# yuanqing-wang/stag

Hardware: NVIDIA B200
Metric: GEdge-samples/s fused stochastic SpMM fwd+bwd (higher is better)
Workload: dtype f32

## Files before the change

stag_b200/csrc/gemm_tcgen05.cu:

```cuda
#include <cuda.h>
#include <stdlib.h>

#include "common.cuh"

namespace stag {

constexpr int GM = 128;
constexpr int GK = 32;
constexpr int GTHREADS = 128;

__device__ __forceinline__ uint32_t smem_u32(const void* p) { return (uint32_t)__cvta_generic_to_shared(p); }

__device__ __forceinline__ float to_tf32(float x) {
  uint32_t y;
  asm("cvt.rna.tf32.f32 %0, %1;" : "=r"(y) : "f"(x));
  return __uint_as_float(y);
}

__device__ __forceinline__ uint64_t make_desc(uint32_t saddr) {
  return (uint64_t)((saddr & 0x3FFFFu) >> 4) | (1ull << 16) | (64ull << 32) | (1ull << 46) | (2ull << 61);
}

__device__ __forceinline__ uint32_t make_idesc(int n) {
  return (1u << 4) | (2u << 7) | (2u << 10) | ((uint32_t)(n >> 3) << 17) | ((uint32_t)(GM >> 4) << 24);
}

__device__ __forceinline__ void mma_tf32(uint32_t tmem_d, uint64_t da, uint64_t db, uint32_t idesc, uint32_t accumulate) {
  asm volatile(
      "{\n\t.reg .pred p;\n\tsetp.ne.b32 p, %4, 0;\n\t"
      "tcgen05.mma.cta_group::1.kind::tf32 [%0], %1, %2, %3, p;\n\t}"
      ::"r"(tmem_d), "l"(da), "l"(db), "r"(idesc), "r"(accumulate)
      : "memory");
}
// ... 490 lines not shown
          const uint32_t s = st.i, l = lo.i;
          mbar_wait_s(FULL(s), st.par);
          if (!lo_first) mbar_wait_s(LO_FREE(l), lo.par ^ 1u);
          st.next();
          lo.next();
          if (lo.i == 0) lo_first = false;
          const uint32_t hi_s = st0 + s * G2_TILE, lo_s = lo0 + l * G2_TILE;
          uint32_t x[8][4];
#pragma unroll
          for (int j = 0; j < 8; ++j) {
            const int idx = lane + 32 * j, r = 32 * w + (idx >> 3), ch = idx & 7;
            const uint32_t o = (uint32_t)r * 128u + (uint32_t)((ch ^ (r & 7)) << 4);
            asm volatile("ld.shared.v4.b32 {%0,%1,%2,%3}, [%4];" : "=r"(x[j][0]), "=r"(x[j][1]), "=r"(x[j][2]), "=r"(x[j][3]) : "r"(hi_s + o));
          }
#pragma unroll
          for (int j = 0; j < 8; ++j) {
            const int idx = lane + 32 * j, r = 32 * w + (idx >> 3), ch = idx & 7;
            const uint32_t o = (uint32_t)r * 128u + (uint32_t)((ch ^ (r & 7)) << 4);
            float l4[4];
#pragma unroll
            for (int t = 0; t < 4; ++t) l4[t] = to_tf32(__uint_as_float(x[j][t]) - __uint_as_float(x[j][t] & 0xFFFFE000u));
            asm volatile("st.shared.v4.f32 [%0], {%1,%2,%3,%4};" ::"r"(lo_s + o), "f"(l4[0]), "f"(l4[1]), "f"(l4[2]), "f"(l4[3]) : "memory");
          }
          asm volatile("fence.proxy.async.shared::cta;" ::: "memory");
          __syncwarp();
          if (lane == 0) mbar_arrive_s(READY(s));
        }
      }
    }
  }
  asm volatile("tcgen05.fence::before_thread_sync;" ::: "memory");
  __syncthreads();
  if (warp == 0) asm volatile("tcgen05.dealloc.cta_group::1.sync.aligned.b32 %0, %1;" ::"r"(tmem_d), "r"(2u * p.ncol) : "memory");
}

typedef CUresult (*EncodeTiledFn)(CUtensorMap*, CUtensorMapDataType, cuuint32_t, void*, const cuuint64_t*, const cuuint64_t*,
                                  const cuuint32_t*, const cuuint32_t*, CUtensorMapInterleave, CUtensorMapSwizzle,
                                  CUtensorMapL2promotion, CUtensorMapFloatOOBfill);
static EncodeTiledFn encode_tiled() {
  static EncodeTiledFn fn = []() -> EncodeTiledFn {
    void* f = nullptr;
    cudaDriverEntryPointQueryResult q;
    if (cudaGetDriverEntryPoint("cuTensorMapEncodeTiled", &f, cudaEnableDefault, &q) != cudaSuccess || q != cudaDriverEntryPointSuccess)
      return nullptr;
    return (EncodeTiledFn)f;
  }();
  return fn;
}

}

using namespace stag;

extern "C" size_t stag_gemm_workspace_bytes(int64_t M, int32_t Nout, int32_t K) {
  (void)M; (void)Nout; (void)K;
  return 0;
}

extern "C" int stag_gemm_tcgen05(const float* a, int64_t lda, const float* wt, int64_t ldw, int64_t M, int32_t Nout,
                                 int32_t K, const float* row_scale, const float* bias, int act, float* out,
                                 int64_t ldo, void* ws, size_t ws_bytes, void* stream_) {
  (void)ws; (void)ws_bytes;
  cudaStream_t stream = (cudaStream_t)stream_;
  STAG_CHECK_ARG(M >= 0 && Nout > 0 && K > 0, "stag_gemm_tcgen05: bad sizes M=%lld N=%d K=%d", (long long)M, Nout, K);
  if (M == 0) return STAG_OK;
  STAG_CHECK_ARG(a && wt && out, "stag_gemm_tcgen05: null argument");
  STAG_CHECK_ARG(lda >= K && ldw >= K && ldo >= Nout, "stag_gemm_tcgen05: leading dimensions too small");
  STAG_CHECK_ARG(act == 0 || act == 1, "stag_gemm_tcgen05: act must be 0 (none) or 1 (relu)");
  if (Nout > 256) {
    set_error("stag_gemm_tcgen05: Nout=%d > 256 output columns per tile are not supported", Nout);
    return STAG_EUNSUPPORTED;
  }
  {
    const int npad2 = (Nout + 15) / 16 * 16, nkb2 = (K + GK - 1) / GK;
    static const char* force1 = getenv("STAG_GEMM_FORM");
    const bool ok = lda % 4 == 0 && (((uintptr_t)a) & 15) == 0 && (size_t)npad2 * nkb2 * 128 * 2 <= 128 * 1024 &&
                    M * lda < (1ll << 40) && !(force1 && atoi(force1) == 1) && encode_tiled() != nullptr;
    if (ok) {
      alignas(64) CUtensorMap tmap;
      const cuuint64_t gdim[2] = {(cuuint64_t)K, (cuuint64_t)M};
// ... 71 lines not shown
```

stag_b200/csrc/spmm.cu:

```cuda
#include <stdlib.h>
#include "common.cuh"
#include "noise.cuh"
#include "param_finalize.cuh"

#ifndef STAG_PACK2
#define STAG_PACK2 1
#endif

namespace stag {

constexpr int AGG_THREADS = 256;
constexpr int AGG_WARPS = AGG_THREADS / 32;

struct AggParams {
  const int32_t* indptr;
  const int32_t* indices;
  const int32_t* eid;
  const int32_t* hub_rows;
  const int32_t* hub_seg_ptr;
  const int32_t* row_order;
  const int32_t* items;
  const int32_t* erow;
  const int32_t* eidf;
  const int4* rec;
  int num_items;
  uint32_t rk[2 * kPhiloxRounds];
  uint32_t kf;
  int num_hubs, num_hub_segs;
  int N;
  int64_t ncols;
  int64_t E;
  const float* x;
  int64_t ldx, x_ss;
  const float* gscale;
  const float* rscale;
// ... 2139 lines not shown
```

stag_b200/csrc/spmm_wq.cuh:

```cuda
#pragma once

namespace stag {

constexpr int WQ_GROUPS = 32, WQ_EPR = 4;
constexpr int WQ_NBUF = 4;
constexpr uint32_t WQ_REC_STRIDE = WQ_NBUF * WQ_EPR * 16 + 16;
constexpr uint32_t WQ_ROW_STRIDE = WQ_NBUF * WQ_EPR * 4 + 4;
__host__ __device__ constexpr uint32_t wq_rec_bytes(int nw) { return (uint32_t)(8 * nw) * WQ_REC_STRIDE; }
__host__ __device__ constexpr uint32_t wq_row_bytes(int nw) { return ((uint32_t)(8 * nw) * WQ_ROW_STRIDE + 15u) & ~15u; }
__host__ __device__ constexpr uint32_t wq_smem(int nw) { return 2 * 128 * 128 + wq_rec_bytes(nw) + wq_row_bytes(nw) + 1024; }

__device__ __forceinline__ void tc_ldtm_16x256b_x8(uint32_t taddr, uint32_t (&v)[32]) {
  asm volatile(
      "tcgen05.ld.sync.aligned.16x256b.x8.b32 "
      "{%0, %1, %2, %3, %4, %5, %6, %7, %8, %9, %10, %11, %12, %13, %14, %15, "
      "%16, %17, %18, %19, %20, %21, %22, %23, %24, %25, %26, %27, %28, %29, %30, %31}, [%32];"
      : "=r"(v[0]), "=r"(v[1]), "=r"(v[2]), "=r"(v[3]), "=r"(v[4]), "=r"(v[5]), "=r"(v[6]), "=r"(v[7]),
        "=r"(v[8]), "=r"(v[9]), "=r"(v[10]), "=r"(v[11]), "=r"(v[12]), "=r"(v[13]), "=r"(v[14]), "=r"(v[15]),
        "=r"(v[16]), "=r"(v[17]), "=r"(v[18]), "=r"(v[19]), "=r"(v[20]), "=r"(v[21]), "=r"(v[22]), "=r"(v[23]),
        "=r"(v[24]), "=r"(v[25]), "=r"(v[26]), "=r"(v[27]), "=r"(v[28]), "=r"(v[29]), "=r"(v[30]), "=r"(v[31])
      : "r"(taddr)
      : "memory");
}
__device__ __forceinline__ void tc_ldtm_wait32(uint32_t (&v)[32]) {
  asm volatile("tcgen05.wait::ld.sync.aligned;"
               : "+r"(v[0]), "+r"(v[1]), "+r"(v[2]), "+r"(v[3]), "+r"(v[4]), "+r"(v[5]), "+r"(v[6]), "+r"(v[7]),
                 "+r"(v[8]), "+r"(v[9]), "+r"(v[10]), "+r"(v[11]), "+r"(v[12]), "+r"(v[13]), "+r"(v[14]), "+r"(v[15]),
                 "+r"(v[16]), "+r"(v[17]), "+r"(v[18]), "+r"(v[19]), "+r"(v[20]), "+r"(v[21]), "+r"(v[22]), "+r"(v[23]),
                 "+r"(v[24]), "+r"(v[25]), "+r"(v[26]), "+r"(v[27]), "+r"(v[28]), "+r"(v[29]), "+r"(v[30]), "+r"(v[31])
               :
               : "memory");
}
__device__ __forceinline__ void tc_ldtm_16x256b_x4(uint32_t taddr, uint32_t (&v)[16]) {
  asm volatile(
      "tcgen05.ld.sync.aligned.16x256b.x4.b32 "
      "{%0, %1, %2, %3, %4, %5, %6, %7, %8, %9, %10, %11, %12, %13, %14, %15}, [%16];"
      : "=r"(v[0]), "=r"(v[1]), "=r"(v[2]), "=r"(v[3]), "=r"(v[4]), "=r"(v[5]), "=r"(v[6]), "=r"(v[7]),
        "=r"(v[8]), "=r"(v[9]), "=r"(v[10]), "=r"(v[11]), "=r"(v[12]), "=r"(v[13]), "=r"(v[14]), "=r"(v[15])
      : "r"(taddr)
      : "memory");
}
__device__ __forceinline__ void tc_ldtm_wait16(uint32_t (&v)[16]) {
  asm volatile("tcgen05.wait::ld.sync.aligned;"
               : "+r"(v[0]), "+r"(v[1]), "+r"(v[2]), "+r"(v[3]), "+r"(v[4]), "+r"(v[5]), "+r"(v[6]), "+r"(v[7]),
                 "+r"(v[8]), "+r"(v[9]), "+r"(v[10]), "+r"(v[11]), "+r"(v[12]), "+r"(v[13]), "+r"(v[14]), "+r"(v[15])
               :
               : "memory");
}
__device__ __forceinline__ void ldg256(const char* src, float4& a, float4& b) {
  asm volatile("ld.global.nc.v8.f32 {%0, %1, %2, %3, %4, %5, %6, %7}, [%8];"
               : "=f"(a.x), "=f"(a.y), "=f"(a.z), "=f"(a.w), "=f"(b.x), "=f"(b.y), "=f"(b.z), "=f"(b.w)
               : "l"(src));
}
__device__ __forceinline__ void stg256cs(char* dst, const float2* v) {
  asm volatile("st.global.cs.v8.f32 [%0], {%1, %2, %3, %4, %5, %6, %7, %8};" ::"l"(dst), "f"(v[0].x), "f"(v[0].y), "f"(v[1].x),
               "f"(v[1].y), "f"(v[2].x), "f"(v[2].y), "f"(v[3].x), "f"(v[3].y)
               : "memory");
}

template <int NW, int XB, bool DB, int MINB, int GMODE = 0, bool LATE_REC = false>
__global__ void __launch_bounds__(32 * NW, MINB) agg_wh_quad_kernel(const AggParams p) {
  constexpr int NCH = 8 / NW;
  constexpr int NU = 2 * NCH;
  constexpr int NBLK = 32 / NW;
  static_assert(NW == 4 || NW == 8, "4 or 8 warps");
  static_assert(NU % XB == 0, "ring slots must be round-invariant");
  extern __shared__ __align__(1024) unsigned char tc_raw[];
  __shared__ uint64_t mma_bar[2];
  __shared__ uint32_t tmem_base_s;
  __shared__ int maxn_s[NW];
  __shared__ int arrive_cnt[2];
  constexpr uint32_t TM_COLS = DB ? 256u : 128u;
  const uint32_t sm0 = ((uint32_t)__cvta_generic_to_shared(tc_raw) + 1023u) & ~1023u;
  const uint32_t h_s = sm0, at_s = sm0 + 128 * 128;
  const int tid = threadIdx.x, warp = tid >> 5, lane = tid & 31;
  const int wq = warp & 3;
  const int ch0 = NW == 8 ? warp >> 2 : 0;
  const int jq = lane >> 2, q = lane & 3;
  const uint32_t rec_base = at_s + 128 * 128, row_base = rec_base + wq_rec_bytes(NW);
  const uint32_t rec_g = rec_base + (uint32_t)(8 * warp + jq) * WQ_REC_STRIDE;
  const uint32_t row_g = row_base + (uint32_t)(8 * warp + jq) * WQ_ROW_STRIDE;
  const uint32_t bar_s = (uint32_t)__cvta_generic_to_shared(mma_bar);
  constexpr uint32_t rmask = WQ_NBUF * WQ_EPR - 1;

  if (warp == 0) {
    asm volatile("tcgen05.alloc.cta_group::1.sync.aligned.shared::cta.b32 [%0], %1;" ::"r"(
                     (uint32_t)__cvta_generic_to_shared(&tmem_base_s)),
                 "r"(TM_COLS)
                 : "memory");
    asm volatile("tcgen05.relinquish_alloc_permit.cta_group::1.sync.aligned;" ::: "memory");
  }
  if (tid == 0) {
    arrive_cnt[0] = arrive_cnt[1] = 0;
    tc_mbar_init(bar_s, 1);
    tc_mbar_init(bar_s + 8, 1);
    asm volatile("fence.mbarrier_init.release.cluster;" ::: "memory");
  }
  for (int n = tid; n < 128; n += 32 * NW) {
    const int kk = n >> 3, qq = (n >> 1) & 3, bb = n & 1;
    const int c = 32 * (kk >> 2) + 8 * qq + 2 * (kk & 3) + bb;
    for (int ch = 0; ch < 8; ++ch) {
      uint32_t wv[4];
#pragma unroll
      for (int w4 = 0; w4 < 4; ++w4) {
        uint32_t word = 0;
#pragma unroll
        for (int b = 0; b < 4; ++b) {
          const int k = ch * 16 + w4 * 4 + b;
          word |= ((__popc(c & k) & 1) ? 0xB8u : 0x38u) << (8 * b);
        }
        wv[w4] = word;
      }
      sts128(h_s + (uint32_t)n * 128u + (uint32_t)((ch ^ (n & 7)) << 4), make_uint4(wv[0], wv[1], wv[2], wv[3]));
    }
  }
  for (uint32_t o = (uint32_t)tid * 16u; o < 128u * 128u; o += 32u * NW * 16u) sts128(at_s + o, make_uint4(0u, 0u, 0u, 0u));
  asm volatile("fence.proxy.async.shared::cta;" ::: "memory");
  asm volatile("tcgen05.fence::before_thread_sync;" ::: "memory");
  __syncthreads();
  asm volatile("tcgen05.fence::after_thread_sync;" ::: "memory");
  const uint32_t tmem0 = tmem_base_s;
  const uint32_t idesc = (1u << 4) | ((uint32_t)(128 >> 3) << 17) | ((uint32_t)(128 >> 4) << 24);
  const uint64_t h_desc = tc_desc(h_s), a_desc = tc_desc(at_s);
  const PhiloxKey key = live_key(p);
  uint32_t mma_count = 0;

  const int G = p.D >> 7;
  const int n_items = p.num_hub_segs + p.num_items;
  const int IG = (n_items + WQ_GROUPS - 1) / WQ_GROUPS;
  const int64_t total = (int64_t)IG * p.S * G;
  const uint32_t ldxb = (uint32_t)p.ldx * 4u, ldo4 = (uint32_t)p.ldo * 4u;
  const int rb = NW == 8 ? 16 * (warp >> 2) : 0;
  const uint32_t mk_rec = rec_base + (uint32_t)(8 * warp + (lane >> 3)) * WQ_REC_STRIDE + 4u;
  const uint32_t mk_row = at_s + (uint32_t)(32 * wq + rb + (lane >> 3)) * 128u;

  __shared__ int item_s;
  int* const queue = reinterpret_cast<int*>(const_cast<int4*>(p.rec) + p.E);
  if (tid == 0) item_s = atomicAdd(queue, 1);
  __syncthreads();
  for (;;) {
    const int64_t item = item_s;
    if (item >= total) break;
    const int64_t outer = item / IG;
    const int gi = (int)(item - outer * IG) * WQ_GROUPS + 8 * wq + jq;
    const int cg = (int)(outer % G), s = (int)(outer / G);
    int e0 = 0, e1 = 0, part_slot = -1;
    if (gi < p.num_hub_segs) {
      int lo = 0, hi = p.num_hubs;
      while (hi - lo > 1) {
        const int mid = (lo + hi) >> 1;
        if (__ldg(p.hub_seg_ptr + mid) <= gi) lo = mid; else hi = mid;
      }
      const int row = __ldg(p.hub_rows + lo);
      const int k = gi - __ldg(p.hub_seg_ptr + lo);
      e0 = __ldg(p.indptr + row) + k * kHubSegment;
      e1 = min(e0 + kHubSegment, __ldg(p.indptr + row + 1));
      part_slot = gi;
    } else if (gi < n_items) {
      const int4 it = __ldg(reinterpret_cast<const int4*>(p.items) + (gi - p.num_hub_segs));
      e0 = it.z;
      e1 = it.w >= 0 ? it.w : it.z;
    }
    const int nedges = e1 - e0;
    const int rowlim = part_slot < 0 ? nedges : 0;
    int maxn = nedges;
#pragma unroll
    for (int o = 16; o > 0; o >>= 1) maxn = max(maxn, __shfl_xor_sync(0xffffffffu, maxn, o));
    __syncthreads();
    if (lane == 0) maxn_s[warp] = maxn;
    if (tid == 0) item_s = atomicAdd(queue, 1);
    __syncthreads();
    maxn = max(max(maxn_s[0], maxn_s[1]), max(maxn_s[2], maxn_s[3]));
    const int rounds = (maxn + WQ_EPR - 1) / WQ_EPR;
    if (rounds == 0) continue;

    const char* xcb = reinterpret_cast<const char*>(p.x + (int64_t)s * p.x_ss + cg * 128 + 64 * ch0 + 8 * q);
    char* outs = reinterpret_cast<char*>(p.out + (int64_t)s * p.out_ss + cg * 128 + 64 * ch0 + 8 * q);
    const uint32_t smp = (uint32_t)(p.sample_base + s);
    const uint32_t blk = (uint32_t)(8 * cg + (lane & 7));
    const int4* recp = p.rec + e0;
    const int32_t* rowp = p.erow + e0;
    float2 acc[8 * NCH];
#pragma unroll
    for (int i = 0; i < 8 * NCH; ++i) acc[i] = make_float2(0.f, 0.f);
    float4 xb[XB][8];

    auto fetch_chunk = [&](int r) {
      const int e = WQ_EPR * r + q;
      const uint32_t pos = (uint32_t)e & rmask;
      const bool off = e >= nedges;
      cp_async16(rec_g + pos * 16u, recp + (off ? 0 : e), off);
      cp_async4(row_g + pos * 4u, rowp + (off ? 0 : e), off);
    };
    auto make_bytes = [&](int r) {
      uint32_t eid[NBLK];
#pragma unroll
      for (int i = 0; i < NBLK; ++i) {
        const int k = (rb + 4 * i) >> 3;
        const uint32_t pos = (uint32_t)(WQ_EPR * r + k) & rmask;
        eid[i] = (uint32_t)lds32(mk_rec + (uint32_t)(4 * (i & 1)) * WQ_REC_STRIDE + (pos << 4));
      }
      uint4 v[NBLK];
#pragma unroll
      for (int i = 0; i < NBLK; ++i) {
        v[i] = philox_rk(blk, eid[i] & 0x7fffffffu, smp, key.c3, p);
        v[i].x = (v[i].x & kWhAnd) | kWhOr; v[i].y = (v[i].y & kWhAnd) | kWhOr;
        v[i].z = (v[i].z & kWhAnd) | kWhOr; v[i].w = (v[i].w & kWhAnd) | kWhOr;
      }
#pragma unroll
      for (int i = 0; i < NBLK; ++i) {
        const int sw = ((lane >> 3) + 4 * (i & 1)) & 7;
        sts128(mk_row + (uint32_t)(4 * i) * 128u + (uint32_t)(((lane & 7) ^ sw) << 4), v[i]);
      }
    };
    auto issue_mma = [&]() {
      const uint32_t buf = DB ? (mma_count & 1u) : 0u;
#pragma unroll
      for (int ks = 0; ks < 4; ++ks)
        tc_mma_f8(tmem0 + buf * 128u, a_desc + (uint64_t)(2 * ks), h_desc + (uint64_t)(2 * ks), idesc, ks != 0);
      asm volatile("tcgen05.commit.cta_group::1.mbarrier::arrive::one.shared::cluster.b64 [%0];" ::"r"(bar_s + 8u * (mma_count & 1u))
                   : "memory");
    };
    auto bytes_and_mma = [&](int r) {
      make_bytes(r);
      asm volatile("fence.proxy.async.shared::cta;" ::: "memory");
      asm volatile("tcgen05.fence::before_thread_sync;" ::: "memory");
      __syncwarp();
      if (lane == 0) {
        uint32_t old;
        const uint32_t cnt_s = (uint32_t)__cvta_generic_to_shared(&arrive_cnt[mma_count & 1u]);
        asm volatile("atom.acq_rel.cta.shared::cta.add.u32 %0, [%1], 1;" : "=r"(old) : "r"(cnt_s) : "memory");
        if (old == NW - 1) {
          asm volatile("st.relaxed.cta.shared::cta.u32 [%0], %1;" ::"r"(cnt_s), "r"(0u) : "memory");
          asm volatile("tcgen05.fence::after_thread_sync;" ::: "memory");
          issue_mma();
        }
      }
      ++mma_count;
    };
    auto load_half = [&](uint32_t un, int chl, float4* dst) {
      const char* src = xcb + (uint64_t)un * ldxb + 256 * chl;
      ldg256(src, dst[0], dst[1]);
      ldg256(src + 128, dst[2], dst[3]);
    };
    auto neighbours = [&](int r, uint32_t (&un)[4]) {
#pragma unroll
      for (int k4 = 0; k4 < 4; ++k4) un[k4] = (uint32_t)lds32(rec_g + (((uint32_t)(WQ_EPR * r + k4) & rmask) << 4));
    };

    fetch_chunk(0);
    fetch_chunk(1);
    cp_async_commit();
    cp_async_wait<0>();
    __syncwarp();
    bytes_and_mma(0);
    uint32_t un1[4];
    {
      uint32_t un0[4];
      neighbours(0, un0);
#pragma unroll
      for (int u = 0; u < XB; ++u) {
        load_half(un0[2 * (u / NCH)], u % NCH, xb[u]);
        load_half(un0[2 * (u / NCH) + 1], u % NCH, xb[u] + 4);
      }
    }

    for (int r = 0; r < rounds; ++r) {
      cp_async_wait<0>();
      __syncwarp();
      fetch_chunk(r + 2);
      cp_async_commit();
      int4 rc4[4];
      uint32_t ro4[4];
      auto read_records = [&]() {
#pragma unroll
        for (int k4 = 0; k4 < 4; ++k4) rc4[k4] = lds128(rec_g + (((uint32_t)(WQ_EPR * r + k4) & rmask) << 4));
#pragma unroll
        for (int k4 = 0; k4 < 4; ++k4) ro4[k4] = (uint32_t)lds32(row_g + (((uint32_t)(WQ_EPR * r + k4) & rmask) << 2));
        neighbours(r + 1, un1);
      };
      if (!LATE_REC) read_records();
      const uint32_t done = mma_count - 1u;
      tc_mbar_wait(bar_s + 8u * (done & 1u), (done >> 1) & 1u);
      asm volatile("tcgen05.fence::after_thread_sync;" ::: "memory");
      const uint32_t taddr = tmem0 + ((uint32_t)(32 * wq) << 16) + (DB ? (done & 1u) * 128u : 0u) + (uint32_t)(64 * ch0);
      if (DB && r + 1 < rounds) bytes_and_mma(r + 1);
      if (LATE_REC) read_records();
#pragma unroll
      for (int u = 0; u < NU; ++u) {
        const int hf = u / NCH, chl = u % NCH;
        uint32_t z[32];
        tc_ldtm_16x256b_x8(taddr + ((uint32_t)(16 * hf) << 16) + (uint32_t)(64 * chl), z);
        float4* xu = xb[u % XB];
        tc_ldtm_wait32(z);
#pragma unroll
        for (int kk = 0; kk < 2; ++kk) {
          const int t = WQ_EPR * r + 2 * hf + kk;
          const int4 rc = rc4[2 * hf + kk];
          if (t < nedges) {
            const float2 AA = make_float2(__int_as_float(rc.z), __int_as_float(rc.z));
            const float2 BB = make_float2(__int_as_float(rc.w), __int_as_float(rc.w));
#pragma unroll
            for (int mm = 0; mm < 2; ++mm) {
              const float xv[8] = {xu[4 * kk + 2 * mm].x, xu[4 * kk + 2 * mm].y, xu[4 * kk + 2 * mm].z, xu[4 * kk + 2 * mm].w,
                                   xu[4 * kk + 2 * mm + 1].x, xu[4 * kk + 2 * mm + 1].y, xu[4 * kk + 2 * mm + 1].z, xu[4 * kk + 2 * mm + 1].w};
#pragma unroll
              for (int e2 = 0; e2 < 4; ++e2) {
                const int zi = 16 * mm + 4 * e2 + 2 * kk;
                const float2 w2 = __ffma2_rn(make_float2(__uint_as_float(z[zi]), __uint_as_float(z[zi + 1])), BB, AA);
                acc[8 * chl + 4 * mm + e2] = __ffma2_rn(w2, make_float2(xv[2 * e2], xv[2 * e2 + 1]), acc[8 * chl + 4 * mm + e2]);
              }
            }
            if (rc.y < 0 && t < rowlim) {
              char* o = outs + ro4[2 * hf + kk] * ldo4 + 256 * chl;
#pragma unroll
              for (int mm = 0; mm < 2; ++mm) {
                stg256cs(o + 128 * mm, acc + 8 * chl + 4 * mm);
#pragma unroll
                for (int e2 = 0; e2 < 4; ++e2) acc[8 * chl + 4 * mm + e2] = make_float2(0.f, 0.f);
              }
            }
          }
          if (GMODE == 0) {
            const int nu = (u + XB) % NU;
            const uint32_t un = (u + XB) < NU ? (uint32_t)rc4[2 * (nu / NCH) + kk].x : un1[2 * (nu / NCH) + kk];
            load_half(un, nu % NCH, xu + 4 * kk);
          }
        }
        if (GMODE == 1) {
#pragma unroll
          for (int kk = 0; kk < 2; ++kk) {
            const int nu = (u + XB) % NU;
            const uint32_t un = (u + XB) < NU ? (uint32_t)rc4[2 * (nu / NCH) + kk].x : un1[2 * (nu / NCH) + kk];
            load_half(un, nu % NCH, xu + 4 * kk);
          }
        }
      }
      if (GMODE == 2) {
        static_assert(GMODE != 2 || XB == NU, "round-end gathers need a whole round in the ring");
#pragma unroll
        for (int u = 0; u < NU; ++u)
#pragma unroll
          for (int kk = 0; kk < 2; ++kk) load_half(un1[2 * (u / NCH) + kk], u % NCH, xb[u] + 4 * kk);
      }
      if (!DB && r + 1 < rounds) {
        asm volatile("tcgen05.fence::before_thread_sync;" ::: "memory");
        bytes_and_mma(r + 1);
      }
    }
    cp_async_wait<0>();
    __syncwarp();
    if (part_slot >= 0) {
      float* o = p.part_acc + ((int64_t)s * p.num_hub_segs + part_slot) * p.dpad + cg * 128 + 64 * ch0 + 8 * q;
#pragma unroll
      for (int m = 0; m < 2 * NCH; ++m) stg256cs(reinterpret_cast<char*>(o + 32 * m), acc + 4 * m);
    }
  }
  zero_empty_rows_tail(p, (int64_t)blockIdx.x * NW + warp, (int64_t)gridDim.x * NW, lane);

  asm volatile("tcgen05.fence::before_thread_sync;" ::: "memory");
  __syncthreads();
  if (warp == 0) asm volatile("tcgen05.dealloc.cta_group::1.sync.aligned.b32 %0, %1;" ::"r"(tmem0), "r"(TM_COLS) : "memory");
}

template <int NW, int XB, bool DB, int MINB, int GMODE = 0, bool LATE_REC = false>
static int launch_wh_quad_inst(const AggParams& p, cudaStream_t stream) {
  const int64_t total = (int64_t)((p.num_hub_segs + p.num_items + WQ_GROUPS - 1) / WQ_GROUPS) * p.S * (p.D >> 7);
  const int64_t cap = (int64_t)num_sms() * MINB;
  const int grid = (int)(total < 1 ? 1 : (total < cap ? total : cap));
  constexpr int max_ctas = DB ? 2 : 4;
  const size_t pad = (size_t)(227 * 1024) / (max_ctas + 1) + 1024;
  const size_t smem = wq_smem(NW) > pad ? wq_smem(NW) : pad;
  STAG_CUDA(cudaFuncSetAttribute(agg_wh_quad_kernel<NW, XB, DB, MINB, GMODE, LATE_REC>, cudaFuncAttributeMaxDynamicSharedMemorySize, (int)smem));
  agg_wh_quad_kernel<NW, XB, DB, MINB, GMODE, LATE_REC><<<grid, 32 * NW, smem, stream>>>(p);
  STAG_LAUNCH_CHECK();
  return STAG_OK;
}

static int launch_wh_quad(const AggParams& p, cudaStream_t stream) {
  if (p.E > 0) {
    edge_record_kernel<STAG_NOISE_NORMAL><<<(unsigned)((p.E + 255) / 256), 256, 0, stream>>>(p, const_cast<int4*>(p.rec), 3);
    STAG_LAUNCH_CHECK();
  } else {
    STAG_CUDA(cudaMemsetAsync(const_cast<int4*>(p.rec), 0, 16, stream));
  }
  STAG_CHECK_ARG((int64_t)((p.num_hub_segs + p.num_items + WQ_GROUPS - 1) / WQ_GROUPS) * p.S * (p.D >> 7) < (1ll << 30),
                 "stag_spmm: too many work items for one launch");
  static const char* var = getenv("STAG_WQ_VARIANT");
  const int v = var ? atoi(var) : 0;
  switch (v) {
    case 1: return launch_wh_quad_inst<4, 4, false, 2, 1>(p, stream);
    case 2: return launch_wh_quad_inst<4, 2, false, 3>(p, stream);
    case 3: return launch_wh_quad_inst<8, 2, true, 2>(p, stream);
    case 4: return launch_wh_quad_inst<4, 4, true, 2, 0>(p, stream);
    case 5: return launch_wh_quad_inst<4, 4, true, 2, 2>(p, stream);
    case 6: return launch_wh_quad_inst<4, 4, true, 2, 1, false>(p, stream);
    case 7: return launch_wh_quad_inst<4, 4, true, 2, 2, true>(p, stream);
    default: return launch_wh_quad_inst<4, 4, true, 2, 1, true>(p, stream);
  }
}

}
```

Measured before the change: 6.885.

## Gather neighbour feature rows with TMA gather4 into shared memory using 8-warp kernel

Replaces the per-thread register-ring global loads of neighbour feature rows with TMA tile::gather4 bulk copies into a swizzled per-warp shared-memory staging area, tracked by per-warp mbarriers. It uses an 8-warp variant where warp pairs share record fetching via named barriers, and only four warps fetch records. The aim is to offload gather address generation and register pressure from the SMs and overlap the gathers with the MMA and accumulation. It adds shared memory use, host-side tensor-map encoding each launch, and a fallback to the 4-warp path, while removing the environment-selected variants.

```diff
diff --git a/stag_b200/csrc/gemm_tcgen05.cu b/stag_b200/csrc/gemm_tcgen05.cu
--- a/stag_b200/csrc/gemm_tcgen05.cu
+++ b/stag_b200/csrc/gemm_tcgen05.cu
@@ -1,4 +1,4 @@
-#include <cuda.h>
+#include "tensor_map.cuh"
 #include <stdlib.h>
 
 #include "common.cuh"
@@ -555,20 +555,6 @@
   asm volatile("tcgen05.fence::before_thread_sync;" ::: "memory");
   __syncthreads();
   if (warp == 0) asm volatile("tcgen05.dealloc.cta_group::1.sync.aligned.b32 %0, %1;" ::"r"(tmem_d), "r"(2u * p.ncol) : "memory");
-}
-
-typedef CUresult (*EncodeTiledFn)(CUtensorMap*, CUtensorMapDataType, cuuint32_t, void*, const cuuint64_t*, const cuuint64_t*,
-                                  const cuuint32_t*, const cuuint32_t*, CUtensorMapInterleave, CUtensorMapSwizzle,
-                                  CUtensorMapL2promotion, CUtensorMapFloatOOBfill);
-static EncodeTiledFn encode_tiled() {
-  static EncodeTiledFn fn = []() -> EncodeTiledFn {
-    void* f = nullptr;
-    cudaDriverEntryPointQueryResult q;
-    if (cudaGetDriverEntryPoint("cuTensorMapEncodeTiled", &f, cudaEnableDefault, &q) != cudaSuccess || q != cudaDriverEntryPointSuccess)
-      return nullptr;
-    return (EncodeTiledFn)f;
-  }();
-  return fn;
 }
 
 }
diff --git a/stag_b200/csrc/spmm.cu b/stag_b200/csrc/spmm.cu
--- a/stag_b200/csrc/spmm.cu
+++ b/stag_b200/csrc/spmm.cu
@@ -1,6 +1,7 @@
 #include <stdlib.h>
 #include "common.cuh"
 #include "noise.cuh"
+#include "tensor_map.cuh"
 #include "param_finalize.cuh"
 
 #ifndef STAG_PACK2
diff --git a/stag_b200/csrc/spmm_wq.cuh b/stag_b200/csrc/spmm_wq.cuh
--- a/stag_b200/csrc/spmm_wq.cuh
+++ b/stag_b200/csrc/spmm_wq.cuh
@@ -6,9 +6,13 @@
 constexpr int WQ_NBUF = 4;
 constexpr uint32_t WQ_REC_STRIDE = WQ_NBUF * WQ_EPR * 16 + 16;
 constexpr uint32_t WQ_ROW_STRIDE = WQ_NBUF * WQ_EPR * 4 + 4;
-__host__ __device__ constexpr uint32_t wq_rec_bytes(int nw) { return (uint32_t)(8 * nw) * WQ_REC_STRIDE; }
-__host__ __device__ constexpr uint32_t wq_row_bytes(int nw) { return ((uint32_t)(8 * nw) * WQ_ROW_STRIDE + 15u) & ~15u; }
-__host__ __device__ constexpr uint32_t wq_smem(int nw) { return 2 * 128 * 128 + wq_rec_bytes(nw) + wq_row_bytes(nw) + 1024; }
+__host__ __device__ constexpr uint32_t wq_rec_bytes() { return 32u * WQ_REC_STRIDE; }
+__host__ __device__ constexpr uint32_t wq_row_bytes() { return (32u * WQ_ROW_STRIDE + 15u) & ~15u; }
+constexpr uint32_t WQ_XROWS = 66;
+__host__ __device__ constexpr uint32_t wq_xrow(int m, int j) { return (uint32_t)(33 * m + 4 * j + (j >= 4 ? 1 : 0)); }
+__host__ __device__ constexpr uint32_t wq_smem(int nw) {
+  return 2 * 128 * 128 + (nw == 8 ? 8u * WQ_XROWS * 128u : 0u) + wq_rec_bytes() + wq_row_bytes() + 1024;
+}
 
 __device__ __forceinline__ void tc_ldtm_16x256b_x8(uint32_t taddr, uint32_t (&v)[32]) {
   asm volatile(
@@ -58,30 +62,44 @@
                : "memory");
 }
 
-template <int NW, int XB, bool DB, int MINB, int GMODE = 0, bool LATE_REC = false>
-__global__ void __launch_bounds__(32 * NW, MINB) agg_wh_quad_kernel(const AggParams p) {
+__device__ __forceinline__ void tma_gather4(uint32_t dst, const CUtensorMap* map, int col, int r0, int r1, int r2, int r3,
+                                            uint32_t bar) {
+  asm volatile(
+      "cp.async.bulk.tensor.2d.shared::cta.global.tile::gather4.mbarrier::complete_tx::bytes [%0], [%1, {%2, %3, %4, %5, %6}], [%7];"
+      ::"r"(dst), "l"(map), "r"(col), "r"(r0), "r"(r1), "r"(r2), "r"(r3), "r"(bar)
+      : "memory");
+}
+
+template <int NW>
+__global__ void __launch_bounds__(32 * NW, 2) agg_wh_quad_kernel(const AggParams p, const __grid_constant__ CUtensorMap xmap,
+                                                                 const int xrow_ss) {
+  constexpr bool SMEM = NW == 8;
   constexpr int NCH = 8 / NW;
   constexpr int NU = 2 * NCH;
   constexpr int NBLK = 32 / NW;
+  constexpr int XB = SMEM ? 1 : 4;
   static_assert(NW == 4 || NW == 8, "4 or 8 warps");
-  static_assert(NU % XB == 0, "ring slots must be round-invariant");
   extern __shared__ __align__(1024) unsigned char tc_raw[];
   __shared__ uint64_t mma_bar[2];
+  __shared__ uint64_t row_bar[NW];
   __shared__ uint32_t tmem_base_s;
   __shared__ int maxn_s[NW];
   __shared__ int arrive_cnt[2];
-  constexpr uint32_t TM_COLS = DB ? 256u : 128u;
+  constexpr uint32_t TM_COLS = 256u;
   const uint32_t sm0 = ((uint32_t)__cvta_generic_to_shared(tc_raw) + 1023u) & ~1023u;
   const uint32_t h_s = sm0, at_s = sm0 + 128 * 128;
   const int tid = threadIdx.x, warp = tid >> 5, lane = tid & 31;
   const int wq = warp & 3;
   const int ch0 = NW == 8 ? warp >> 2 : 0;
   const int jq = lane >> 2, q = lane & 3;
-  const uint32_t rec_base = at_s + 128 * 128, row_base = rec_base + wq_rec_bytes(NW);
-  const uint32_t rec_g = rec_base + (uint32_t)(8 * warp + jq) * WQ_REC_STRIDE;
-  const uint32_t row_g = row_base + (uint32_t)(8 * warp + jq) * WQ_ROW_STRIDE;
+  const uint32_t xrow_base = at_s + 128 * 128 + (uint32_t)warp * WQ_XROWS * 128u;
+  const uint32_t rec_base = at_s + 128 * 128 + (SMEM ? 8u * WQ_XROWS * 128u : 0u), row_base = rec_base + wq_rec_bytes();
+  const uint32_t rec_g = rec_base + (uint32_t)(8 * wq + jq) * WQ_REC_STRIDE;
+  const uint32_t row_g = row_base + (uint32_t)(8 * wq + jq) * WQ_ROW_STRIDE;
   const uint32_t bar_s = (uint32_t)__cvta_generic_to_shared(mma_bar);
+  const uint32_t rbar = (uint32_t)__cvta_generic_to_shared(&row_bar[warp]);
   constexpr uint32_t rmask = WQ_NBUF * WQ_EPR - 1;
+  const bool fetcher = !SMEM || warp < 4;
 
   if (warp == 0) {
     asm volatile("tcgen05.alloc.cta_group::1.sync.aligned.shared::cta.b32 [%0], %1;" ::"r"(
@@ -94,6 +112,8 @@
     arrive_cnt[0] = arrive_cnt[1] = 0;
     tc_mbar_init(bar_s, 1);
     tc_mbar_init(bar_s + 8, 1);
+    if (SMEM)
+      for (int w = 0; w < NW; ++w) tc_mbar_init((uint32_t)__cvta_generic_to_shared(&row_bar[w]), 1);
     asm volatile("fence.mbarrier_init.release.cluster;" ::: "memory");
   }
   for (int n = tid; n < 128; n += 32 * NW) {
@@ -124,6 +144,7 @@
   const uint64_t h_desc = tc_desc(h_s), a_desc = tc_desc(at_s);
   const PhiloxKey key = live_key(p);
   uint32_t mma_count = 0;
+  uint32_t row_count = 0;
 
   const int G = p.D >> 7;
   const int n_items = p.num_hub_segs + p.num_items;
@@ -131,8 +152,11 @@
   const int64_t total = (int64_t)IG * p.S * G;
   const uint32_t ldxb = (uint32_t)p.ldx * 4u, ldo4 = (uint32_t)p.ldo * 4u;
   const int rb = NW == 8 ? 16 * (warp >> 2) : 0;
-  const uint32_t mk_rec = rec_base + (uint32_t)(8 * warp + (lane >> 3)) * WQ_REC_STRIDE + 4u;
+  const uint32_t mk_rec = rec_base + (uint32_t)(8 * wq + (lane >> 3)) * WQ_REC_STRIDE + 4u;
   const uint32_t mk_row = at_s + (uint32_t)(32 * wq + rb + (lane >> 3)) * 128u;
+  auto pair_sync = [&]() {
+    if (SMEM) asm volatile("bar.sync %0, 64;" ::"r"(1 + wq) : "memory");
+  };
 
   __shared__ int item_s;
   int* const queue = reinterpret_cast<int*>(const_cast<int4*>(p.rec) + p.E);
@@ -214,7 +238,7 @@
       }
     };
     auto issue_mma = [&]() {
-      const uint32_t buf = DB ? (mma_count & 1u) : 0u;
+      const uint32_t buf = mma_count & 1u;
 #pragma unroll
       for (int ks = 0; ks < 4; ++ks)
         tc_mma_f8(tmem0 + buf * 128u, a_desc + (uint64_t)(2 * ks), h_desc + (uint64_t)(2 * ks), idesc, ks != 0);
@@ -243,49 +267,76 @@
       ldg256(src, dst[0], dst[1]);
       ldg256(src + 128, dst[2], dst[3]);
     };
+    const int xrow0 = s * xrow_ss, xcol = cg * 128 + 64 * ch0;
+    auto gather_round = [&](const uint32_t (&un)[4]) {
+      __syncwarp();
+      if (lane == 0)
+        asm volatile("mbarrier.arrive.expect_tx.shared::cta.b64 _, [%0], %1;" ::"r"(rbar), "r"(8u * 4u * 2u * 128u) : "memory");
+      __syncwarp();
+      if (q == 0) {
+#pragma unroll
+        for (int m = 0; m < 2; ++m)
+          tma_gather4(xrow_base + wq_xrow(m, jq) * 128u, &xmap, xcol + 32 * m, xrow0 + (int)un[0], xrow0 + (int)un[1],
+                      xrow0 + (int)un[2], xrow0 + (int)un[3], rbar);
+      }
+    };
     auto neighbours = [&](int r, uint32_t (&un)[4]) {
 #pragma unroll
       for (int k4 = 0; k4 < 4; ++k4) un[k4] = (uint32_t)lds32(rec_g + (((uint32_t)(WQ_EPR * r + k4) & rmask) << 4));
     };
 
-    fetch_chunk(0);
-    fetch_chunk(1);
-    cp_async_commit();
-    cp_async_wait<0>();
+    if (fetcher) {
+      fetch_chunk(0);
+      fetch_chunk(1);
+      cp_async_commit();
+      cp_async_wait<0>();
+    }
     __syncwarp();
+    pair_sync();
     bytes_and_mma(0);
     uint32_t un1[4];
     {
       uint32_t un0[4];
       neighbours(0, un0);
-#pragma unroll
-      for (int u = 0; u < XB; ++u) {
-        load_half(un0[2 * (u / NCH)], u % NCH, xb[u]);
-        load_half(un0[2 * (u / NCH) + 1], u % NCH, xb[u] + 4);
+      if (SMEM) {
+#ifndef WQ_KO_GATHER
+        gather_round(un0);
+#endif
+      } else {
+#pragma unroll
+        for (int u = 0; u < XB; ++u) {
+          load_half(un0[2 * (u / NCH)], u % NCH, xb[u]);
+          load_half(un0[2 * (u / NCH) + 1], u % NCH, xb[u] + 4);
+        }
       }
     }
 
     for (int r = 0; r < rounds; ++r) {
-      cp_async_wait<0>();
+      if (fetcher) cp_async_wait<0>();
       __syncwarp();
-      fetch_chunk(r + 2);
-      cp_async_commit();
+      pair_sync();
+      if (fetcher) {
+        fetch_chunk(r + 2);
+        cp_async_commit();
+      }
       int4 rc4[4];
       uint32_t ro4[4];
-      auto read_records = [&]() {
-#pragma unroll
-        for (int k4 = 0; k4 < 4; ++k4) rc4[k4] = lds128(rec_g + (((uint32_t)(WQ_EPR * r + k4) & rmask) << 4));
-#pragma unroll
-        for (int k4 = 0; k4 < 4; ++k4) ro4[k4] = (uint32_t)lds32(row_g + (((uint32_t)(WQ_EPR * r + k4) & rmask) << 2));
-        neighbours(r + 1, un1);
-      };
-      if (!LATE_REC) read_records();
       const uint32_t done = mma_count - 1u;
       tc_mbar_wait(bar_s + 8u * (done & 1u), (done >> 1) & 1u);
       asm volatile("tcgen05.fence::after_thread_sync;" ::: "memory");
-      const uint32_t taddr = tmem0 + ((uint32_t)(32 * wq) << 16) + (DB ? (done & 1u) * 128u : 0u) + (uint32_t)(64 * ch0);
-      if (DB && r + 1 < rounds) bytes_and_mma(r + 1);
-      if (LATE_REC) read_records();
+      const uint32_t taddr = tmem0 + ((uint32_t)(32 * wq) << 16) + (done & 1u) * 128u + (uint32_t)(64 * ch0);
+      if (r + 1 < rounds) bytes_and_mma(r + 1);
+#pragma unroll
+      for (int k4 = 0; k4 < 4; ++k4) rc4[k4] = lds128(rec_g + (((uint32_t)(WQ_EPR * r + k4) & rmask) << 4));
+#pragma unroll
+      for (int k4 = 0; k4 < 4; ++k4) ro4[k4] = (uint32_t)lds32(row_g + (((uint32_t)(WQ_EPR * r + k4) & rmask) << 2));
+      neighbours(r + 1, un1);
+      if (SMEM) {
+#ifndef WQ_KO_GATHER
+        tc_mbar_wait(rbar, row_count & 1u);
+#endif
+        ++row_count;
+      }
 #pragma unroll
       for (int u = 0; u < NU; ++u) {
         const int hf = u / NCH, chl = u % NCH;
@@ -302,8 +353,21 @@
             const float2 BB = make_float2(__int_as_float(rc.w), __int_as_float(rc.w));
 #pragma unroll
             for (int mm = 0; mm < 2; ++mm) {
-              const float xv[8] = {xu[4 * kk + 2 * mm].x, xu[4 * kk + 2 * mm].y, xu[4 * kk + 2 * mm].z, xu[4 * kk + 2 * mm].w,
-                                   xu[4 * kk + 2 * mm + 1].x, xu[4 * kk + 2 * mm + 1].y, xu[4 * kk + 2 * mm + 1].z, xu[4 * kk + 2 * mm + 1].w};
+              float4 x0, x1;
+              if (SMEM) {
+                const uint32_t row = xrow_base + (wq_xrow(mm, jq) + (uint32_t)(2 * hf + kk)) * 128u;
+                const uint32_t ph = (row >> 7) & 7u;
+#ifdef WQ_KO_LDS
+                x0 = x1 = make_float4(AA.x, BB.x, __uint_as_float(row), AA.y);
+#else
+                x0 = lds128f(row + (((2u * q) ^ ph) << 4));
+                x1 = lds128f(row + (((2u * q + 1u) ^ ph) << 4));
+#endif
+              } else {
+                x0 = xu[4 * kk + 2 * mm];
+                x1 = xu[4 * kk + 2 * mm + 1];
+              }
+              const float xv[8] = {x0.x, x0.y, x0.z, x0.w, x1.x, x1.y, x1.z, x1.w};
 #pragma unroll
               for (int e2 = 0; e2 < 4; ++e2) {
                 const int zi = 16 * mm + 4 * e2 + 2 * kk;
@@ -321,34 +385,17 @@
               }
             }
           }
-          if (GMODE == 0) {
-            const int nu = (u + XB) % NU;
-            const uint32_t un = (u + XB) < NU ? (uint32_t)rc4[2 * (nu / NCH) + kk].x : un1[2 * (nu / NCH) + kk];
-            load_half(un, nu % NCH, xu + 4 * kk);
-          }
         }
-        if (GMODE == 1) {
-#pragma unroll
-          for (int kk = 0; kk < 2; ++kk) {
-            const int nu = (u + XB) % NU;
-            const uint32_t un = (u + XB) < NU ? (uint32_t)rc4[2 * (nu / NCH) + kk].x : un1[2 * (nu / NCH) + kk];
-            load_half(un, nu % NCH, xu + 4 * kk);
-          }
+        if (!SMEM) {
+#pragma unroll
+          for (int kk = 0; kk < 2; ++kk) load_half(un1[2 * (u / NCH) + kk], u % NCH, xu + 4 * kk);
         }
       }
-      if (GMODE == 2) {
-        static_assert(GMODE != 2 || XB == NU, "round-end gathers need a whole round in the ring");
-#pragma unroll
-        for (int u = 0; u < NU; ++u)
-#pragma unroll
-          for (int kk = 0; kk < 2; ++kk) load_half(un1[2 * (u / NCH) + kk], u % NCH, xb[u] + 4 * kk);
-      }
-      if (!DB && r + 1 < rounds) {
-        asm volatile("tcgen05.fence::before_thread_sync;" ::: "memory");
-        bytes_and_mma(r + 1);
-      }
-    }
-    cp_async_wait<0>();
+#ifndef WQ_KO_GATHER
+      if (SMEM && r + 1 < rounds) gather_round(un1);
+#endif
+    }
+    if (fetcher) cp_async_wait<0>();
     __syncwarp();
     if (part_slot >= 0) {
       float* o = p.part_acc + ((int64_t)s * p.num_hub_segs + part_slot) * p.dpad + cg * 128 + 64 * ch0 + 8 * q;
@@ -363,18 +410,40 @@
   if (warp == 0) asm volatile("tcgen05.dealloc.cta_group::1.sync.aligned.b32 %0, %1;" ::"r"(tmem0), "r"(TM_COLS) : "memory");
 }
 
-template <int NW, int XB, bool DB, int MINB, int GMODE = 0, bool LATE_REC = false>
-static int launch_wh_quad_inst(const AggParams& p, cudaStream_t stream) {
+template <int NW>
+static int launch_wh_quad_inst(const AggParams& p, const CUtensorMap& xmap, int xrow_ss, cudaStream_t stream) {
   const int64_t total = (int64_t)((p.num_hub_segs + p.num_items + WQ_GROUPS - 1) / WQ_GROUPS) * p.S * (p.D >> 7);
-  const int64_t cap = (int64_t)num_sms() * MINB;
+  const int64_t cap = (int64_t)num_sms() * 2;
   const int grid = (int)(total < 1 ? 1 : (total < cap ? total : cap));
-  constexpr int max_ctas = DB ? 2 : 4;
-  const size_t pad = (size_t)(227 * 1024) / (max_ctas + 1) + 1024;
+  const size_t pad = (size_t)(227 * 1024) / 3 + 1024;
   const size_t smem = wq_smem(NW) > pad ? wq_smem(NW) : pad;
-  STAG_CUDA(cudaFuncSetAttribute(agg_wh_quad_kernel<NW, XB, DB, MINB, GMODE, LATE_REC>, cudaFuncAttributeMaxDynamicSharedMemorySize, (int)smem));
-  agg_wh_quad_kernel<NW, XB, DB, MINB, GMODE, LATE_REC><<<grid, 32 * NW, smem, stream>>>(p);
+  STAG_CUDA(cudaFuncSetAttribute(agg_wh_quad_kernel<NW>, cudaFuncAttributeMaxDynamicSharedMemorySize, (int)smem));
+  agg_wh_quad_kernel<NW><<<grid, 32 * NW, smem, stream>>>(p, xmap, xrow_ss);
   STAG_LAUNCH_CHECK();
   return STAG_OK;
+}
+
+static bool wq_tensor_map(const AggParams& p, CUtensorMap* map, int* xrow_ss) {
+  if (p.x_ss % p.ldx != 0) return false;
+  const int64_t ss = p.x_ss / p.ldx;
+  const int64_t rows = ss * (p.S - 1) + p.ncols;
+  if (rows >= (1ll << 31) || p.ldx * 4 >= (1ll << 40) || encode_tiled() == nullptr) return false;
+  static const bool fits = [] {
+    int n = 0;
+    return cudaFuncSetAttribute(agg_wh_quad_kernel<8>, cudaFuncAttributeMaxDynamicSharedMemorySize, (int)wq_smem(8)) == cudaSuccess &&
+           cudaOccupancyMaxActiveBlocksPerMultiprocessor(&n, agg_wh_quad_kernel<8>, 256, wq_smem(8)) == cudaSuccess && n >= 2;
+  }();
+  if (!fits) return false;
+  const cuuint64_t gdim[2] = {(cuuint64_t)p.D, (cuuint64_t)rows};
+  const cuuint64_t gstr[1] = {(cuuint64_t)p.ldx * 4};
+  const cuuint32_t box[2] = {32, 1};
+  const cuuint32_t estr[2] = {1, 1};
+  if (encode_tiled()(map, CU_TENSOR_MAP_DATA_TYPE_FLOAT32, 2, const_cast<float*>(p.x), gdim, gstr, box, estr,
+                     CU_TENSOR_MAP_INTERLEAVE_NONE, CU_TENSOR_MAP_SWIZZLE_128B, CU_TENSOR_MAP_L2_PROMOTION_L2_128B,
+                     CU_TENSOR_MAP_FLOAT_OOB_FILL_NONE) != CUDA_SUCCESS)
+    return false;
+  *xrow_ss = (int)ss;
+  return true;
 }
 
 static int launch_wh_quad(const AggParams& p, cudaStream_t stream) {
@@ -386,18 +455,11 @@
   }
   STAG_CHECK_ARG((int64_t)((p.num_hub_segs + p.num_items + WQ_GROUPS - 1) / WQ_GROUPS) * p.S * (p.D >> 7) < (1ll << 30),
                  "stag_spmm: too many work items for one launch");
-  static const char* var = getenv("STAG_WQ_VARIANT");
-  const int v = var ? atoi(var) : 0;
-  switch (v) {
-    case 1: return launch_wh_quad_inst<4, 4, false, 2, 1>(p, stream);
-    case 2: return launch_wh_quad_inst<4, 2, false, 3>(p, stream);
-    case 3: return launch_wh_quad_inst<8, 2, true, 2>(p, stream);
-    case 4: return launch_wh_quad_inst<4, 4, true, 2, 0>(p, stream);
-    case 5: return launch_wh_quad_inst<4, 4, true, 2, 2>(p, stream);
-    case 6: return launch_wh_quad_inst<4, 4, true, 2, 1, false>(p, stream);
-    case 7: return launch_wh_quad_inst<4, 4, true, 2, 2, true>(p, stream);
-    default: return launch_wh_quad_inst<4, 4, true, 2, 1, true>(p, stream);
-  }
-}
-
-}
+  alignas(64) CUtensorMap xmap;
+  int xrow_ss = 0;
+  if (wq_tensor_map(p, &xmap, &xrow_ss)) return launch_wh_quad_inst<8>(p, xmap, xrow_ss, stream);
+  memset(&xmap, 0, sizeof xmap);
+  return launch_wh_quad_inst<4>(p, xmap, 0, stream);
+}
+
+}
diff --git a/stag_b200/csrc/tensor_map.cuh b/stag_b200/csrc/tensor_map.cuh
--- /dev/null
+++ b/stag_b200/csrc/tensor_map.cuh
@@ -0,0 +1,21 @@
+#pragma once
+#include <cuda.h>
+#include <cuda_runtime.h>
+
+namespace stag {
+
+typedef CUresult (*EncodeTiledFn)(CUtensorMap*, CUtensorMapDataType, cuuint32_t, void*, const cuuint64_t*, const cuuint64_t*,
+                                  const cuuint32_t*, const cuuint32_t*, CUtensorMapInterleave, CUtensorMapSwizzle,
+                                  CUtensorMapL2promotion, CUtensorMapFloatOOBfill);
+static EncodeTiledFn encode_tiled() {
+  static EncodeTiledFn fn = []() -> EncodeTiledFn {
+    void* f = nullptr;
+    cudaDriverEntryPointQueryResult q;
+    if (cudaGetDriverEntryPoint("cuTensorMapEncodeTiled", &f, cudaEnableDefault, &q) != cudaSuccess || q != cudaDriverEntryPointSuccess)
+      return nullptr;
+    return (EncodeTiledFn)f;
+  }();
+  return fn;
+}
+
+}
```

New measurement: 6.787, median of 6. -1.4%, worse.

## Stage gathered feature rows through a cp.async shared-memory ring with paired warps

Applied to the files above, without the earlier changes.

Adds an SRING mode to the warp-quad SpMM kernel. Gathered x rows are staged through a shared-memory ring filled by cp.async instead of register float4 buffers. With 8 warps, warp pairs share one edge-record buffer synchronised by named barriers, so only one warp of each pair fetches records. The default variant switches to this 8-warp shared-ring configuration. The aim is to cut register pressure and overlap gathers asynchronously, at the cost of extra shared-memory traffic, barriers and a larger shared-memory footprint per CTA.

```diff
diff --git a/stag_b200/csrc/spmm_wq.cuh b/stag_b200/csrc/spmm_wq.cuh
--- a/stag_b200/csrc/spmm_wq.cuh
+++ b/stag_b200/csrc/spmm_wq.cuh
@@ -1,4 +1,8 @@
 #pragma once
+
+#ifndef STAG_WQ_KO
+#define STAG_WQ_KO 0
+#endif
 
 namespace stag {
 
@@ -8,7 +12,10 @@
 constexpr uint32_t WQ_ROW_STRIDE = WQ_NBUF * WQ_EPR * 4 + 4;
 __host__ __device__ constexpr uint32_t wq_rec_bytes(int nw) { return (uint32_t)(8 * nw) * WQ_REC_STRIDE; }
 __host__ __device__ constexpr uint32_t wq_row_bytes(int nw) { return ((uint32_t)(8 * nw) * WQ_ROW_STRIDE + 15u) & ~15u; }
-__host__ __device__ constexpr uint32_t wq_smem(int nw) { return 2 * 128 * 128 + wq_rec_bytes(nw) + wq_row_bytes(nw) + 1024; }
+__host__ __device__ constexpr uint32_t wq_ring_bytes(int xb) { return (uint32_t)(2 * xb) * 4u * 256u * 16u; }
+__host__ __device__ constexpr uint32_t wq_smem(int nrec, uint32_t ring = 0) {
+  return 2 * 128 * 128 + wq_rec_bytes(nrec) + wq_row_bytes(nrec) + ring + 1024;
+}
 
 __device__ __forceinline__ void tc_ldtm_16x256b_x8(uint32_t taddr, uint32_t (&v)[32]) {
   asm volatile(
@@ -58,13 +65,16 @@
                : "memory");
 }
 
-template <int NW, int XB, bool DB, int MINB, int GMODE = 0, bool LATE_REC = false>
+template <int NW, int XB, bool DB, int MINB, int GMODE = 0, bool LATE_REC = false, bool SRING = false>
 __global__ void __launch_bounds__(32 * NW, MINB) agg_wh_quad_kernel(const AggParams p) {
   constexpr int NCH = 8 / NW;
   constexpr int NU = 2 * NCH;
   constexpr int NBLK = 32 / NW;
   static_assert(NW == 4 || NW == 8, "4 or 8 warps");
   static_assert(NU % XB == 0, "ring slots must be round-invariant");
+  static_assert(!SRING || NW == 8, "the shared-memory ring is laid out for 256 threads");
+  constexpr bool PAIR = SRING && XB == NU;
+  constexpr int NREC = PAIR ? 4 : NW;
   extern __shared__ __align__(1024) unsigned char tc_raw[];
   __shared__ uint64_t mma_bar[2];
   __shared__ uint32_t tmem_base_s;
@@ -77,9 +87,14 @@
   const int wq = warp & 3;
   const int ch0 = NW == 8 ? warp >> 2 : 0;
   const int jq = lane >> 2, q = lane & 3;
-  const uint32_t rec_base = at_s + 128 * 128, row_base = rec_base + wq_rec_bytes(NW);
-  const uint32_t rec_g = rec_base + (uint32_t)(8 * warp + jq) * WQ_REC_STRIDE;
-  const uint32_t row_g = row_base + (uint32_t)(8 * warp + jq) * WQ_ROW_STRIDE;
+  const uint32_t rec_base = at_s + 128 * 128, row_base = rec_base + wq_rec_bytes(NREC);
+  const int rw = PAIR ? wq : warp;
+  const uint32_t rec_g = rec_base + (uint32_t)(8 * rw + jq) * WQ_REC_STRIDE;
+  const uint32_t row_g = row_base + (uint32_t)(8 * rw + jq) * WQ_ROW_STRIDE;
+  const float4* const xs = reinterpret_cast<const float4*>(tc_raw + (sm0 - (uint32_t)__cvta_generic_to_shared(tc_raw)) + 2 * 128 * 128 +
+                                                           wq_rec_bytes(NREC) + wq_row_bytes(NREC)) + tid;
+  const uint32_t xs_s = (uint32_t)__cvta_generic_to_shared(xs);
+  const uint32_t xs_q = xs_s + (uint32_t)((lane & 1) * 4096 + ((lane & 3) >> 1) * 16) - (uint32_t)((lane & 3) * 16);
   const uint32_t bar_s = (uint32_t)__cvta_generic_to_shared(mma_bar);
   constexpr uint32_t rmask = WQ_NBUF * WQ_EPR - 1;
 
@@ -131,7 +146,7 @@
   const int64_t total = (int64_t)IG * p.S * G;
   const uint32_t ldxb = (uint32_t)p.ldx * 4u, ldo4 = (uint32_t)p.ldo * 4u;
   const int rb = NW == 8 ? 16 * (warp >> 2) : 0;
-  const uint32_t mk_rec = rec_base + (uint32_t)(8 * warp + (lane >> 3)) * WQ_REC_STRIDE + 4u;
+  const uint32_t mk_rec = rec_base + (uint32_t)(8 * rw + (lane >> 3)) * WQ_REC_STRIDE + 4u;
   const uint32_t mk_row = at_s + (uint32_t)(32 * wq + rb + (lane >> 3)) * 128u;
 
   __shared__ int item_s;
@@ -186,6 +201,7 @@
     float4 xb[XB][8];
 
     auto fetch_chunk = [&](int r) {
+      if (PAIR && ch0 != 0) return;
       const int e = WQ_EPR * r + q;
       const uint32_t pos = (uint32_t)e & rmask;
       const bool off = e >= nedges;
@@ -247,12 +263,23 @@
 #pragma unroll
       for (int k4 = 0; k4 < 4; ++k4) un[k4] = (uint32_t)lds32(rec_g + (((uint32_t)(WQ_EPR * r + k4) & rmask) << 4));
     };
+    auto rec_sync = [&]() {
+      if (PAIR) asm volatile("bar.sync %0, 64;" ::"r"(1 + wq) : "memory");
+      else __syncwarp();
+    };
+    auto ring_fill = [&](int k, uint32_t un, int t) {
+      const bool off = t >= nedges;
+      const char* src = xcb - 16 * q + (off ? 0 : (uint64_t)un * ldxb);
+#pragma unroll
+      for (int pc = 0; pc < 4; ++pc)
+        if (STAG_WQ_KO < 2) cp_async16(xs_q + (uint32_t)((4 * k + 2 * (pc >> 1)) * 4096 + 32 * (pc & 1)), src + 128 * (pc >> 1) + 64 * (pc & 1), off);
+    };
 
     fetch_chunk(0);
     fetch_chunk(1);
     cp_async_commit();
     cp_async_wait<0>();
-    __syncwarp();
+    rec_sync();
     bytes_and_mma(0);
     uint32_t un1[4];
     {
@@ -260,14 +287,20 @@
       neighbours(0, un0);
 #pragma unroll
       for (int u = 0; u < XB; ++u) {
-        load_half(un0[2 * (u / NCH)], u % NCH, xb[u]);
-        load_half(un0[2 * (u / NCH) + 1], u % NCH, xb[u] + 4);
+        if constexpr (SRING) {
+          ring_fill(2 * u, un0[2 * u], 2 * u);
+          ring_fill(2 * u + 1, un0[2 * u + 1], 2 * u + 1);
+          cp_async_commit();
+        } else {
+          load_half(un0[2 * (u / NCH)], u % NCH, xb[u]);
+          load_half(un0[2 * (u / NCH) + 1], u % NCH, xb[u] + 4);
+        }
       }
     }
 
     for (int r = 0; r < rounds; ++r) {
-      cp_async_wait<0>();
-      __syncwarp();
+      if constexpr (SRING) cp_async_wait<XB>(); else cp_async_wait<0>();
+      rec_sync();
       fetch_chunk(r + 2);
       cp_async_commit();
       int4 rc4[4];
@@ -292,6 +325,12 @@
         uint32_t z[32];
         tc_ldtm_16x256b_x8(taddr + ((uint32_t)(16 * hf) << 16) + (uint32_t)(64 * chl), z);
         float4* xu = xb[u % XB];
+        if constexpr (SRING) {
+          if (XB == NU) cp_async_wait<2>();
+          else if (u == 0) cp_async_wait<1>();
+          else cp_async_wait<0>();
+          __syncwarp();
+        }
         tc_ldtm_wait32(z);
 #pragma unroll
         for (int kk = 0; kk < 2; ++kk) {
@@ -302,8 +341,16 @@
             const float2 BB = make_float2(__int_as_float(rc.w), __int_as_float(rc.w));
 #pragma unroll
             for (int mm = 0; mm < 2; ++mm) {
-              const float xv[8] = {xu[4 * kk + 2 * mm].x, xu[4 * kk + 2 * mm].y, xu[4 * kk + 2 * mm].z, xu[4 * kk + 2 * mm].w,
-                                   xu[4 * kk + 2 * mm + 1].x, xu[4 * kk + 2 * mm + 1].y, xu[4 * kk + 2 * mm + 1].z, xu[4 * kk + 2 * mm + 1].w};
+              const int xk = 4 * (2 * (u % XB) + kk) + 2 * mm;
+              const float4 xa = SRING ? xs[256 * xk] : xu[4 * kk + 2 * mm];
+              const float4 xc = SRING ? xs[256 * (xk + 1)] : xu[4 * kk + 2 * mm + 1];
+              const float xv[8] = {xa.x, xa.y, xa.z, xa.w, xc.x, xc.y, xc.z, xc.w};
+#if STAG_WQ_KO
+              if (SRING) {
+                asm volatile("" ::"f"(xv[0]), "f"(xv[1]), "f"(xv[2]), "f"(xv[3]), "f"(xv[4]), "f"(xv[5]), "f"(xv[6]), "f"(xv[7]));
+                continue;
+              }
+#endif
 #pragma unroll
               for (int e2 = 0; e2 < 4; ++e2) {
                 const int zi = 16 * mm + 4 * e2 + 2 * kk;
@@ -311,7 +358,7 @@
                 acc[8 * chl + 4 * mm + e2] = __ffma2_rn(w2, make_float2(xv[2 * e2], xv[2 * e2 + 1]), acc[8 * chl + 4 * mm + e2]);
               }
             }
-            if (rc.y < 0 && t < rowlim) {
+            if (rc.y < 0 && t < rowlim && !(STAG_WQ_KO && SRING)) {
               char* o = outs + ro4[2 * hf + kk] * ldo4 + 256 * chl;
 #pragma unroll
               for (int mm = 0; mm < 2; ++mm) {
@@ -321,13 +368,22 @@
               }
             }
           }
-          if (GMODE == 0) {
+          if (GMODE == 0 && !SRING) {
             const int nu = (u + XB) % NU;
             const uint32_t un = (u + XB) < NU ? (uint32_t)rc4[2 * (nu / NCH) + kk].x : un1[2 * (nu / NCH) + kk];
             load_half(un, nu % NCH, xu + 4 * kk);
           }
         }
-        if (GMODE == 1) {
+        if constexpr (SRING) {
+          __syncwarp();
+          const int nu = (u + XB) % NU;
+#pragma unroll
+          for (int kk = 0; kk < 2; ++kk) {
+            const uint32_t un = (u + XB) < NU ? (uint32_t)rc4[2 * nu + kk].x : un1[2 * nu + kk];
+            ring_fill(2 * (u % XB) + kk, un, WQ_EPR * (r + (u + XB) / NU) + 2 * nu + kk);
+          }
+          cp_async_commit();
+        } else if (GMODE == 1) {
 #pragma unroll
           for (int kk = 0; kk < 2; ++kk) {
             const int nu = (u + XB) % NU;
@@ -336,7 +392,7 @@
           }
         }
       }
-      if (GMODE == 2) {
+      if (GMODE == 2 && !SRING) {
         static_assert(GMODE != 2 || XB == NU, "round-end gathers need a whole round in the ring");
 #pragma unroll
         for (int u = 0; u < NU; ++u)
@@ -363,16 +419,19 @@
   if (warp == 0) asm volatile("tcgen05.dealloc.cta_group::1.sync.aligned.b32 %0, %1;" ::"r"(tmem0), "r"(TM_COLS) : "memory");
 }
 
-template <int NW, int XB, bool DB, int MINB, int GMODE = 0, bool LATE_REC = false>
+template <int NW, int XB, bool DB, int MINB, int GMODE = 0, bool LATE_REC = false, bool SRING = false>
 static int launch_wh_quad_inst(const AggParams& p, cudaStream_t stream) {
   const int64_t total = (int64_t)((p.num_hub_segs + p.num_items + WQ_GROUPS - 1) / WQ_GROUPS) * p.S * (p.D >> 7);
   const int64_t cap = (int64_t)num_sms() * MINB;
   const int grid = (int)(total < 1 ? 1 : (total < cap ? total : cap));
+  constexpr int nrec = SRING && XB == 2 ? 4 : NW;
+  constexpr uint32_t need = wq_smem(nrec, SRING ? wq_ring_bytes(XB) : 0u);
   constexpr int max_ctas = DB ? 2 : 4;
   const size_t pad = (size_t)(227 * 1024) / (max_ctas + 1) + 1024;
-  const size_t smem = wq_smem(NW) > pad ? wq_smem(NW) : pad;
-  STAG_CUDA(cudaFuncSetAttribute(agg_wh_quad_kernel<NW, XB, DB, MINB, GMODE, LATE_REC>, cudaFuncAttributeMaxDynamicSharedMemorySize, (int)smem));
-  agg_wh_quad_kernel<NW, XB, DB, MINB, GMODE, LATE_REC><<<grid, 32 * NW, smem, stream>>>(p);
+  const size_t smem = need > pad ? need : pad;
+  static_assert((size_t)(max_ctas) * (need + 2048) <= 228 * 1024, "the shared-memory request admits fewer CTAs than TMEM");
+  STAG_CUDA(cudaFuncSetAttribute(agg_wh_quad_kernel<NW, XB, DB, MINB, GMODE, LATE_REC, SRING>, cudaFuncAttributeMaxDynamicSharedMemorySize, (int)smem));
+  agg_wh_quad_kernel<NW, XB, DB, MINB, GMODE, LATE_REC, SRING><<<grid, 32 * NW, smem, stream>>>(p);
   STAG_LAUNCH_CHECK();
   return STAG_OK;
 }
@@ -389,15 +448,10 @@
   static const char* var = getenv("STAG_WQ_VARIANT");
   const int v = var ? atoi(var) : 0;
   switch (v) {
-    case 1: return launch_wh_quad_inst<4, 4, false, 2, 1>(p, stream);
-    case 2: return launch_wh_quad_inst<4, 2, false, 3>(p, stream);
-    case 3: return launch_wh_quad_inst<8, 2, true, 2>(p, stream);
-    case 4: return launch_wh_quad_inst<4, 4, true, 2, 0>(p, stream);
-    case 5: return launch_wh_quad_inst<4, 4, true, 2, 2>(p, stream);
-    case 6: return launch_wh_quad_inst<4, 4, true, 2, 1, false>(p, stream);
-    case 7: return launch_wh_quad_inst<4, 4, true, 2, 2, true>(p, stream);
-    default: return launch_wh_quad_inst<4, 4, true, 2, 1, true>(p, stream);
-  }
-}
-
-}
+    case 1: return launch_wh_quad_inst<4, 4, true, 2, 1, true>(p, stream);
+    case 2: return launch_wh_quad_inst<8, 1, true, 2, 1, true, true>(p, stream);
+    default: return launch_wh_quad_inst<8, 2, true, 2, 1, true, true>(p, stream);
+  }
+}
+
+}
```

After: 6.861 before, 2.808 after, median of 6. -59.1%, worse.
